# WesleyHsieh0806/TAO-Amodal

Hardware: AMD Instinct MI355X
Metric: box-pair IoU+match throughput (higher is better)
Workload: dtype f64

## Files before the change

### include/tao_amodal_hip.h

```cpp
#ifndef TAO_AMODAL_HIP_H
#define TAO_AMODAL_HIP_H

#include <stddef.h>
#include <stdint.h>

#ifdef __cplusplus
extern "C" {
#endif

#define TAOAMD_N_THR 10
#define TAOAMD_N_REC 101
#define TAOAMD_LVIS_RNG 6
#define TAOAMD_TAO_RNG 20

#define TAOAMD_GT_IGNORE 1
#define TAOAMD_GT_OOF 2
#define TAOAMD_GT_ID_HIDDEN 4
#define TAOAMD_DT_IGNORE_UNMATCHED 1
#define TAOAMD_DT_NO_CONSUME 2

#define TAOAMD_OK 0
#define TAOAMD_ERR_HIP 1
#define TAOAMD_ERR_ARG 2
#define TAOAMD_ERR_TOO_LARGE 3
// ... 59 lines not shown
                          const int32_t *gt_frame_pos, int64_t gt_frames,
                          int64_t gt_total, const int64_t *gt_off,
                          const uint32_t *gt_runs, const int32_t *gt_hw,
                          int32_t mode, double *iou,
                          int64_t *pair_frames, void *workspace,
                          size_t workspace_bytes, void *stream);

int taoamd_track_iou(int64_t n_cells, const int32_t *cell_dt_off,
                     const int32_t *cell_gt_off, const int64_t *cell_iou_off,
                     int64_t n_pairs, const int32_t *dt_frame_off,
                     const int32_t *dt_frame_pos, const double *dt_frame_box,
                     const int32_t *gt_frame_off, const int32_t *gt_frame_pos,
                     const double *gt_frame_box, int32_t mode, double *iou,
                     int64_t *pair_frames, void *stream);
int taoamd_track_iou_planned(int64_t n_tasks, const int32_t *tasks,
                             const int32_t *task_rows, const int32_t *task_pairs,
                             const int64_t *task_out, const double *frames,
                             const int32_t *task_base, const int32_t *trk_meta,
                             int32_t mode, double *iou, int64_t *pair_frames,
                             int64_t n_zero, const int64_t *zero_out,
                             void *stream);

int taoamd_track_iou_single(int64_t n_dt, const int32_t *dt_group,
                            const int64_t *cell_iou_off, const int32_t *dt_frame_pos,
                            const double *dt_frame_box, const int32_t *gt_frame_pos,
                            const double *gt_frame_box, int32_t mode, double *iou,
                            int64_t *pair_frames, void *stream);

int taoamd_track_pad(int64_t n_trk, int64_t n_frames, const int32_t *frame_off,
                     const int32_t *frame_pos, const double *frame_box,
                     const int32_t *meta, int64_t slot_first, int64_t n_slots,
                     double *padded, int32_t *inexact, void *stream);

int taoamd_track_stream(int64_t n_tasks, const int32_t *tasks,
                        const int32_t *task_rows, const int32_t *trk_meta,
                        const int32_t *task_base, const double *padded,
                        double *frames, void *stream);

int taoamd_track_iou_near(int64_t n_cells, const int32_t *cell_gt_off,
                          const int64_t *cell_iou_off, int64_t n_pairs,
                          const double *iou, int32_t max_ulp, int32_t capacity,
                          int32_t *count, int64_t *list, void *stream);

int64_t taoamd_track_iou_setorder_table(int64_t max_dt_frames, int64_t max_gt_frames);
int taoamd_track_iou_setorder(
    int64_t n_cells, const int32_t *cell_dt_off, const int32_t *cell_gt_off,
    const int64_t *cell_iou_off, const int32_t *cell_unit, const int64_t *tl_vid_start,
    const int64_t *tl_image_id, const int32_t *dt_frame_off, const int32_t *dt_frame_pos,
    const double *dt_frame_box, const int32_t *gt_frame_off, const int32_t *gt_frame_pos,
    const double *gt_frame_box, int32_t mode, const int32_t *count, int32_t capacity,
// ... 8 lines not shown
                                  const int64_t *b, int64_t *out, int64_t *n_out);

int taoamd_track_iou_plan_host(int64_t n_cells, const int32_t *cell_dt_off_host,
                               const int32_t *cell_gt_off_host,
                               const int64_t *cell_iou_off_host,
                               const int32_t *trk_meta_host, int64_t *sizes,
                               int32_t *tasks_host, int32_t *task_rows_host,
                               int32_t *task_pairs_host, int64_t *task_out_host);
int taoamd_track_iou_plan_spans_host(int64_t n_cells, const int32_t *cell_dt_off_host,
                                     const int32_t *cell_gt_off_host,
                                     const int64_t *cell_iou_off_host,
                                     const int32_t *trk_meta_host, int64_t *sizes,
                                     int32_t *tasks_host, int32_t *task_rows_host,
                                     int32_t *task_pairs_host, int64_t *task_out_host,
                                     int64_t *zero_out_host);

#define TAOAMD_MAX_GT_PER_CELL 3072
int taoamd_match(int64_t n_cells, const int32_t *cell_dt_off,
                 const int32_t *cell_gt_off, const int64_t *cell_iou_off,
                 int32_t max_gt_per_cell, const double *dt_box,
                 const double *gt_box, const double *iou, int32_t n_rng,
                 const uint32_t *gt_rng, const uint32_t *dt_rng,
                 const uint8_t *gt_flags, const uint8_t *dt_flags,
                 const int32_t *dst, int64_t out_stride, uint64_t *matched,
                 uint64_t *ignored, int32_t *match_gt, double *ious_out,
                 const int32_t *dt_group, const uint32_t *dt_meta,
                 const int32_t *groups, int32_t n_groups, const int32_t *singles,
                 int32_t n_singles, void *stream);

int taoamd_match_compact(int64_t n_cells, const int32_t *cell_dt_off,
// ... 422 lines not shown
```

### tao_amodal_amd/csrc/api.hip

```cpp
#include <stdio.h>
#include <string.h>

#include <map>
#include <mutex>
#include <string>
#include <vector>

#include "common.hpp"

namespace taoamd {

static thread_local char g_err[512] = "";

void set_error(hipError_t e, const char *what)
{
    snprintf(g_err, sizeof(g_err), "%s: %s", what, hipGetErrorString(e));
}

static void fill(double *out, double start, double stop, int num)
{
    const double step = (stop - start) / (double)(num - 1);
    for (int i = 0; i < num; i++) out[i] = (double)i * step + start;
    out[num - 1] = stop;
}
// ... 163 lines not shown

extern "C" const char *taoamd_strerror(int status)
{
    switch (status) {
    case TAOAMD_OK: return "ok";
    case TAOAMD_ERR_HIP: return "HIP runtime error (see taoamd_last_error)";
    case TAOAMD_ERR_ARG: return "bad argument";
    case TAOAMD_ERR_TOO_LARGE: return "a cell exceeds a kernel limit";
    case TAOAMD_ERR_WORKSPACE: return "workspace too small";
    }
    return "unknown status";
}

extern "C" const char *taoamd_last_error(void) { return taoamd::g_err; }

extern "C" int taoamd_version(void) { return 110; }

extern "C" int taoamd_thresholds_host(double *iou_thrs, double *rec_thrs)
{
    if (!iou_thrs || !rec_thrs) return TAOAMD_ERR_ARG;
    const IouThr i = taoamd::default_iou();
    const RecThr r = taoamd::default_rec();
    memcpy(iou_thrs, i.v, sizeof(double) * N_THR);
    memcpy(rec_thrs, r.v, sizeof(double) * N_REC);
    return TAOAMD_OK;
}

extern "C" int taoamd_set_thresholds(const double *iou_thrs, const double *rec_thrs)
{
    using namespace taoamd;
    IouThr i = default_iou();
// ... 40 lines not shown
```

### tao_amodal_amd/csrc/track_iou.hip

```cpp
#include <algorithm>
#include <vector>

#include "common.hpp"
#include "pyset.hpp"

using namespace taoamd;

__device__ __forceinline__ int64_t find_cell(const int64_t *__restrict__ off,
                                             int64_t n_cells, int64_t p)
{
    int64_t lo = 0, hi = n_cells;
    while (hi - lo > 1) {
        int64_t mid = (lo + hi) >> 1;
        if (off[mid] <= p) lo = mid; else hi = mid;
    }
    return lo;
}

struct FrameQueue {
    const int32_t *__restrict__ pos;
    const double4 *__restrict__ box;
    int32_t p, e;
    int32_t f0, f1, f2;
    double4 b0, b1, b2;
// ... 113 lines not shown
    }
    if (pair_frames != nullptr) {
        __shared__ unsigned long long s_common[4];
        for (int s = WAVE / 2; s > 0; s >>= 1)
            common += __shfl_down(common, s, WAVE);
        if (lane_id() == 0) s_common[threadIdx.x >> 6] = common;
        __syncthreads();
        if (threadIdx.x == 0) {
            const unsigned long long t = s_common[0] + s_common[1] + s_common[2] + s_common[3];
            if (t) atomicAdd(pair_frames, t);
        }
    }
}

#define TT_P 8
#define TT_ROWS 32
#define TT_RS (5 * TT_P + 2)
#define TT_GROUPS (64 / TT_P)
#define TT_ROUNDS ((TT_ROWS + TT_GROUPS - 1) / TT_GROUPS)
#define TT_SLOTS (TT_ROUNDS * TT_GROUPS)
#define TT_FAR 1e300
#define TT_SETS 2
#define TT_ZERO_PER 8

__device__ __forceinline__ double tt_max(double a, double b)
{
    double r;
    asm("v_max_f64 %0, %1, %2" : "=v"(r) : "v"(a), "v"(b));
    return r;
}
__device__ __forceinline__ double tt_min(double a, double b)
// ... 5 lines not shown
__device__ __forceinline__ double tt_pos(double a)
{
    double r;
    asm("v_max_f64 %0, %1, 0" : "=v"(r) : "v"(a));
    return r;
}

__device__ __forceinline__ void tt_barrier()
{
    asm volatile("s_waitcnt lgkmcnt(0)\n\ts_barrier" ::: "memory");
}

template <int S, bool MASKS>
__device__ __forceinline__ void tt_stager(
    const double4 *__restrict__ frames, int64_t sbase, double (*rows)[TT_ROWS * TT_RS],
    const int4 *meta, int32_t p_first, int n_chunks, int lane)
{
    constexpr int NR = (TT_ROUNDS - S + 1) / 2;
    const int grp = lane / TT_P, j = lane % TT_P;
    uint32_t bit[NR];
#pragma unroll
    for (int i = 0; i < NR; i++) bit[i] = 1u << (TT_GROUPS * (S + 2 * i) + grp);
    static_assert(TT_SLOTS <= 32, "one 32-bit mask of a task's rows");
    const int4 mrow = meta[lane & (TT_SLOTS - 1)];
    const uint32_t has_rows = (uint32_t)__builtin_amdgcn_ballot_w64(lane < TT_SLOTS && mrow.y >= mrow.x);
    double4 B[TT_SETS][NR];
    uint32_t pmv[TT_SETS];
    const char *const tbase = reinterpret_cast<const char *>(frames + sbase);
    uint32_t cur = 0;
    const uint32_t joff = (uint32_t)j * 32u;

    auto issue = [&](double4 *Bx, uint32_t &pm_set, int32_t pc) {
        const uint32_t pm = (uint32_t)(__builtin_amdgcn_ballot_w64(mrow.x < pc + TT_P) &
                                       __builtin_amdgcn_ballot_w64(mrow.y >= pc)) & has_rows;
        pm_set = pm;
#pragma unroll
        for (int i = 0; i < NR; i++) {
            const uint32_t off = cur + ((uint32_t)__popc(pm & (bit[i] - 1u)) << 8) + joff;
#ifdef TT_ABLATE_LOADS
            Bx[i] = *reinterpret_cast<const double4 *>(tbase + (off & 0u));
#elif defined(TT_ABLATE_CACHED)
            Bx[i] = *reinterpret_cast<const double4 *>(
                reinterpret_cast<const char *>(frames) + (((uint32_t)(sbase * 32) + off) & 0xfffe0u));
#else
            Bx[i] = *reinterpret_cast<const double4 *>(tbase + off);
#endif
        }
        cur += (uint32_t)__popc(pm) << 8;
    };
// ... 28 lines not shown
    for (int k = 0; k < n_chunks; k += TT_SETS) {
#pragma unroll
        for (int a = 1; a <= TT_SETS; a++) {
            const int c = k + a;
            if (c - 1 >= n_chunks) break;
            if (c < n_chunks) stage(B[a % TT_SETS], pmv[a % TT_SETS], a & 1);
            issue(B[a % TT_SETS], pmv[a % TT_SETS], p_first + (c + TT_SETS) * TT_P);
            tt_barrier();
        }
    }
}

template <int MODE, bool COUNT = true>
__global__ __launch_bounds__(192) __attribute__((amdgpu_waves_per_eu(MODE == 2 ? 4 : 6, MODE == 2 ? 4 : 6))) void track_iou_task_kernel(
    const int4 *__restrict__ tasks, const int32_t *__restrict__ task_rows,
    const int32_t *__restrict__ task_pairs, const int64_t *__restrict__ task_out,
    const double4 *__restrict__ frames, const int32_t *__restrict__ task_base,
    const int4 *__restrict__ trk_meta,
    double *__restrict__ iou, unsigned long long *__restrict__ pair_frames,
    int32_t n_tasks, int64_t n_zero, const int64_t *__restrict__ zero_out)
{
    __shared__ __align__(16) double rows[2][TT_ROWS * TT_RS];
    __shared__ int4 meta[TT_SLOTS];
    __shared__ int32_t span[2];

    if ((int32_t)blockIdx.x >= n_tasks) {
        const int64_t stride = (int64_t)(gridDim.x - n_tasks) * blockDim.x;
        for (int64_t k = (int64_t)(blockIdx.x - n_tasks) * blockDim.x + threadIdx.x;
             k < n_zero; k += stride)
            iou[zero_out[k]] = 0.0;
        return;
    }

    const int lane = threadIdx.x & 63;
    const int wave = threadIdx.x >> 6;
    const bool stager = wave < 2;
    const int4 tk = tasks[blockIdx.x];
    const int n_rows = tk.y, n_pairs = tk.w;

    if (wave == 0) {
        int32_t p_lo = INT32_MAX, p_hi = -1;
        if (lane < TT_SLOTS) {
            int4 m = make_int4(INT32_MAX, -1, 0, 0);
            if (lane < n_rows) m = trk_meta[task_rows[tk.x + lane]];
            if (m.y >= m.x) {
                p_lo = m.x;
                p_hi = m.y;
            } else {
                m.x = INT32_MAX;
                m.y = -1;
            }
            meta[lane] = m;
        }
#pragma unroll
        for (int s = 32; s > 0; s >>= 1) {
            p_lo = min(p_lo, __shfl_xor(p_lo, s));
            p_hi = max(p_hi, __shfl_xor(p_hi, s));
        }
        if (lane == 0) {
            span[0] = p_lo & ~(TT_P - 1);
            span[1] = p_hi;
        }
    }
    __syncthreads();
    const int32_t p_first = span[0], p_hi = span[1];
    const int n_chunks = p_hi < 0 ? 0 : (p_hi - p_first) / TT_P + 1;

    if (stager) {
        const int64_t sbase = (int64_t)task_base[blockIdx.x] * TT_P;
        constexpr bool MASKS = MODE != 0 || COUNT;
        if (wave == 0)
            tt_stager<0, MASKS>(frames, sbase, rows, meta, p_first, n_chunks, lane);
        else
            tt_stager<1, MASKS>(frames, sbase, rows, meta, p_first, n_chunks, lane);
        return;
    }

    int32_t pr = 0;
    if (lane < n_pairs) pr = task_pairs[tk.z + lane];
    const int rowd = pr & 0xFF, rowg = (pr >> 8) & 0xFF;
    int32_t Fd = INT32_MAX, Ld = -1, Fg = INT32_MAX, Lg = -1;
    if (lane < n_pairs) {
        const int4 md = meta[rowd], mg = meta[rowg];
        Fd = md.x;
        Ld = md.y;
        Fg = mg.x;
        Lg = mg.y;
    }
    const int offd = rowd * (TT_RS * 8), offg = rowg * (TT_RS * 8);
    double u = 0.0, i = 0.0;
    unsigned long long common = 0;
    auto add = [&](int b, int32_t pc) {
#ifdef TT_ABLATE_ADDER
        return;
#endif
        const bool dp = Fd < pc + TT_P && Ld >= pc;
        const bool gp = Fg < pc + TT_P && Lg >= pc;
        if (__ballot(dp || gp) == 0) return;
// ... 184 lines not shown
        const pyset::Frames D{dfpos + dfoff[td], dfbox + 4 * (int64_t)dfoff[td],
                              dfoff[td + 1] - dfoff[td]};
        const pyset::Frames Gf{gfpos + gfoff[tg], gfbox + 4 * (int64_t)gfoff[tg],
                               gfoff[tg + 1] - gfoff[tg]};
        if (pyset::table_size(4ull * ((uint64_t)D.n + Gf.n)) > table_cap) {
            atomicOr(status, 1);
            continue;
        }
        iou[p] = pyset::set_order_iou(tl_image_id + tl_vid_start[cell_unit[c]], D, Gf,
                                      mode, buf, table_cap);
    }
}

__global__ __launch_bounds__(TT_SLOTS * TT_P) void track_stream_kernel(
    const int4 *__restrict__ tasks, const int32_t *__restrict__ task_rows,
    const int4 *__restrict__ trk_meta, const int32_t *__restrict__ task_base,
    const double4 *__restrict__ padded, double4 *__restrict__ out)
{
    __shared__ int4 meta[TT_SLOTS];
    const int4 tk = tasks[blockIdx.x];
    const int tid = threadIdx.x;
    if (tid < TT_SLOTS)
        meta[tid] = tid < tk.y ? trk_meta[task_rows[tk.x + tid]] : make_int4(INT32_MAX, -1, 0, 0);
    if (blockIdx.x == 0 && tid < TT_P) out[tid] = make_double4(TT_FAR, TT_FAR, 0.0, 0.0);
    __syncthreads();
    int32_t p_lo = INT32_MAX, p_hi = -1;
    for (int r = 0; r < TT_SLOTS; r++) {
        const int4 m = meta[r];
        if (m.y >= m.x) {
            p_lo = min(p_lo, m.x);
            p_hi = max(p_hi, m.y);
        }
    }
    if (p_hi < 0) return;
    const int r = tid / TT_P, j = tid % TT_P;
    const int4 mine = meta[r];
    const bool has = mine.y >= mine.x;
    int64_t cursor = (int64_t)task_base[blockIdx.x] * TT_P;
    for (int32_t pc = p_lo & ~(TT_P - 1); pc <= p_hi; pc += TT_P) {
        uint32_t pm = 0;
        for (int q = 0; q < TT_SLOTS; q++) {
            const int4 m = meta[q];
            if (m.y >= m.x && m.x < pc + TT_P && m.y >= pc) pm |= 1u << q;
        }
        if (has && ((pm >> r) & 1u)) {
            const int32_t p = pc + j;
            const bool in = p >= mine.x && p <= mine.y;
            out[cursor + (__popc(pm & ((1u << r) - 1u)) * TT_P + j)] =
                in ? padded[(int64_t)mine.z + p] : make_double4(TT_FAR, TT_FAR, 0.0, 0.0);
        }
        cursor += __popc(pm) * TT_P;
    }
}

__global__ void track_pad_fill_kernel(int64_t n, double4 *__restrict__ padded)
{
    const int64_t k = blockIdx.x * (int64_t)blockDim.x + threadIdx.x;
    if (k < n) padded[k] = make_double4(TT_FAR, TT_FAR, 0.0, 0.0);
}

extern "C" int taoamd_track_iou(int64_t n_cells, const int32_t *cell_dt_off,
                                const int32_t *cell_gt_off,
                                const int64_t *cell_iou_off, int64_t n_pairs,
                                const int32_t *dt_frame_off,
                                const int32_t *dt_frame_pos,
                                const double *dt_frame_box,
// ... 28 lines not shown
    if (n_dt == 0) return TAOAMD_OK;
    if (!dt_group || !cell_iou_off || !dt_frame_pos || !dt_frame_box || !gt_frame_pos ||
        !gt_frame_box || !iou)
        return TAOAMD_ERR_ARG;
    TAO_TIMED("track_iou_single_kernel", s,
              track_iou_single_kernel<<<(unsigned)std::min<int64_t>((n_dt + 255) / 256, 2048), 256, 0, s>>>(
                  n_dt, (const int4 *)dt_group, cell_iou_off, dt_frame_pos,
                  (const double4 *)dt_frame_box, gt_frame_pos, (const double4 *)gt_frame_box,
                  iou, (unsigned long long *)pair_frames, mode));
    TAO_LAUNCH_CHECK();
    return TAOAMD_OK;
}

extern "C" int taoamd_track_iou_planned(int64_t n_tasks, const int32_t *tasks,
                                        const int32_t *task_rows,
                                        const int32_t *task_pairs,
                                        const int64_t *task_out,
                                        const double *frames,
                                        const int32_t *task_base,
                                        const int32_t *trk_meta, int32_t mode,
                                        double *iou, int64_t *pair_frames,
                                        int64_t n_zero, const int64_t *zero_out,
                                        void *stream)
{
    hipStream_t s = (hipStream_t)stream;
    if (mode < 0 || mode > 2 || n_tasks < 0 || n_tasks > INT32_MAX - 4096 || n_zero < 0 ||
        (n_zero > 0 && !zero_out))
        return TAOAMD_ERR_ARG;
    if (pair_frames) TAO_HIP(hipMemsetAsync(pair_frames, 0, 8, s));
    if (n_tasks == 0 && n_zero == 0) return TAOAMD_OK;
    if (!iou || (n_tasks > 0 && (!tasks || !task_rows || !task_pairs || !task_out || !frames ||
                                 !task_base || !trk_meta)))
        return TAOAMD_ERR_ARG;
    unsigned long long *pf = (unsigned long long *)pair_frames;
    const unsigned zero_wgs = (unsigned)std::min<int64_t>(
        (n_zero + 192 * TT_ZERO_PER - 1) / (192 * TT_ZERO_PER), 4096);
    const unsigned grid = (unsigned)n_tasks + zero_wgs;
    static const unsigned lds_pad = getenv("TAOAMD_TT_LDS_PAD") ? (unsigned)atoi(getenv("TAOAMD_TT_LDS_PAD")) : 0u;
#define TT_LAUNCH(M)                                                           \
    TAO_TIMED("track_iou_task_kernel", s,                                      \
              track_iou_task_kernel<M><<<grid, 192, lds_pad, s>>>(             \
                  (const int4 *)tasks, task_rows, task_pairs, task_out,        \
                  (const double4 *)frames, task_base, (const int4 *)trk_meta, iou, pf, \
                  (int32_t)n_tasks, n_zero, zero_out))
    if (mode == 0 && pf == nullptr)
        TAO_TIMED("track_iou_task_kernel", s,
                  (track_iou_task_kernel<0, false><<<grid, 192, lds_pad, s>>>(
                      (const int4 *)tasks, task_rows, task_pairs, task_out,
                      (const double4 *)frames, task_base, (const int4 *)trk_meta, iou, pf,
                      (int32_t)n_tasks, n_zero, zero_out)));
    else if (mode == 0) TT_LAUNCH(0);
    else if (mode == 1) TT_LAUNCH(1);
    else TT_LAUNCH(2);
#undef TT_LAUNCH
    TAO_LAUNCH_CHECK();
    return TAOAMD_OK;
}

extern "C" int taoamd_track_pad(int64_t n_trk, int64_t n_frames,
                                const int32_t *frame_off,
                                const int32_t *frame_pos,
                                const double *frame_box, const int32_t *meta,
                                int64_t slot_first, int64_t n_slots,
// ... 7 lines not shown
        TAO_TIMED("track_pad_fill_kernel", s, track_pad_fill_kernel<<<(unsigned)((n_slots + 255) / 256), 256, 0, s>>>(
            n_slots, (double4 *)padded + slot_first));
    }
    if (n_frames > 0) {
        if (!frame_off || !frame_pos || !frame_box || !meta || !padded)
            return TAOAMD_ERR_ARG;
        TAO_TIMED("track_pad_kernel", s, track_pad_kernel<<<(unsigned)((n_frames + 255) / 256), 256, 0, s>>>(
            n_frames, n_trk, frame_off, frame_pos, (const double4 *)frame_box,
            (const int4 *)meta, (double4 *)padded, inexact));
    }
    TAO_LAUNCH_CHECK();
    return TAOAMD_OK;
}

extern "C" int taoamd_track_stream(int64_t n_tasks, const int32_t *tasks,
                                   const int32_t *task_rows, const int32_t *trk_meta,
                                   const int32_t *task_base, const double *padded,
                                   double *frames, void *stream)
{
    hipStream_t s = (hipStream_t)stream;
    if (n_tasks < 0) return TAOAMD_ERR_ARG;
    if (n_tasks == 0) return TAOAMD_OK;
    if (!tasks || !task_rows || !trk_meta || !task_base || !padded || !frames)
        return TAOAMD_ERR_ARG;
    TAO_TIMED("track_stream_kernel", s,
              track_stream_kernel<<<(unsigned)n_tasks, TT_SLOTS * TT_P, 0, s>>>(
                  (const int4 *)tasks, task_rows, (const int4 *)trk_meta, task_base,
                  (const double4 *)padded, (double4 *)frames));
    TAO_LAUNCH_CHECK();
    return TAOAMD_OK;
}

extern "C" int taoamd_track_iou_near(int64_t n_cells, const int32_t *cell_gt_off,
                                     const int64_t *cell_iou_off, int64_t n_pairs,
                                     const double *iou, int32_t max_ulp,
                                     int32_t capacity, int32_t *count,
                                     int64_t *list, void *stream)
{
    hipStream_t s = (hipStream_t)stream;
    if (n_cells < 0 || n_pairs < 0 || max_ulp < 0 || capacity < 0 || !count)
        return TAOAMD_ERR_ARG;
    TAO_HIP(hipMemsetAsync(count, 0, sizeof(int32_t), s));
// ... 85 lines not shown
    }
    const uint32_t cap = pyset::table_size(4ull * (uint64_t)(n_a + n_b));
    std::vector<int32_t> buf(3 * (size_t)cap);
    auto hash = [&](int32_t c) { return (uint64_t)keys[c - 1]; };
    auto ca = [&](uint32_t k) { return code[k]; };
    auto cb = [&](uint32_t k) { return code[n_a + k]; };
    const pyset::Set R = pyset::set_union((uint32_t)n_a, ca, (uint32_t)n_b, cb, hash,
                                          buf.data(), cap);
    int64_t n = 0;
    for (uint32_t i = 0; i <= R.mask; i++)
        if (R.t[i]) out[n++] = keys[R.t[i] - 1];
    *n_out = n;
    return TAOAMD_OK;
}

static int tt_plan(bool spans, int64_t n_cells, const int32_t *cell_dt_off,
                   const int32_t *cell_gt_off, const int64_t *cell_iou_off,
                   const int32_t *trk_meta, int64_t *sizes, int32_t *tasks,
                   int32_t *task_rows, int32_t *task_pairs, int64_t *task_out,
                   int64_t *zero_out)
{
    if (n_cells < 0 || !cell_dt_off || !cell_gt_off || !cell_iou_off ||
        !trk_meta || !sizes)
        return TAOAMD_ERR_ARG;
    const bool fill = tasks != nullptr;
    if (fill && (!task_rows || !task_pairs || !task_out)) return TAOAMD_ERR_ARG;
    const int64_t n_dt = cell_dt_off[n_cells];
    auto first_of = [&](int64_t t) { return trk_meta[4 * t]; };
    auto last_of = [&](int64_t t) { return trk_meta[4 * t + 1]; };
    auto zero_pair = [&](int64_t d, int64_t g) {
// ... 19 lines not shown
        for (int64_t c = 0; c < n_cells; c++) {
            if (cell_hi[c] < 0) continue;
            const int32_t d0 = cell_dt_off[c], D = cell_dt_off[c + 1] - d0;
            const int32_t g0 = cell_gt_off[c], G = cell_gt_off[c + 1] - g0;
            for (int32_t d = 0; d < D; d++)
                for (int32_t g = 0; g < G; g++)
                    if (zero_pair(d0 + d, n_dt + g0 + g)) {
                        if (zero_out) zero_out[nz] = cell_iou_off[c] + (int64_t)d * G + g;
                        nz++;
                    }
        }
    std::stable_sort(order.begin(), order.end(), [&](int64_t a, int64_t b) {
        return cell_hi[a] > cell_hi[b];
    });
    int64_t nt = 0, nr = 0, np = 0;
    int32_t rows[TT_ROWS], n_rows = 0, n_pairs = 0;
    int32_t pair_d[64], pair_g[64];
    int64_t pair_out[64];
    auto close = [&]() {
        if (n_pairs == 0) { n_rows = 0; return; }
        if (fill) {
            int32_t perm[TT_ROWS], inv[TT_ROWS];
            for (int r = 0; r < n_rows; r++) perm[r] = r;
            std::stable_sort(perm, perm + n_rows, [&](int32_t a, int32_t b) {
                return first_of(rows[a]) < first_of(rows[b]);
            });
            for (int r = 0; r < n_rows; r++) inv[perm[r]] = r;
            tasks[4 * nt] = (int32_t)nr;
            tasks[4 * nt + 1] = n_rows;
            tasks[4 * nt + 2] = (int32_t)np;
            tasks[4 * nt + 3] = n_pairs;
            for (int r = 0; r < n_rows; r++) task_rows[nr + r] = rows[perm[r]];
            for (int k = 0; k < n_pairs; k++) {
                task_pairs[np + k] = inv[pair_d[k]] | (inv[pair_g[k]] << 8);
                task_out[np + k] = pair_out[k];
            }
        }
        nt++;
        nr += n_rows;
        np += n_pairs;
        n_rows = n_pairs = 0;
    };
    std::vector<int32_t> dts;
    for (int64_t c : order) {
        const int32_t d0 = cell_dt_off[c], D = cell_dt_off[c + 1] - d0;
        const int32_t g0 = cell_gt_off[c], G = cell_gt_off[c + 1] - g0;
        dts.resize(D);
        for (int32_t d = 0; d < D; d++) dts[d] = d;
        std::stable_sort(dts.begin(), dts.end(), [&](int32_t a, int32_t b) {
            return first_of(d0 + a) < first_of(d0 + b);
        });
        const int32_t gblocks = (G + TT_ROWS - 2) / (TT_ROWS - 1);
        for (int32_t gb = 0; gb < gblocks; gb++) {
            const int32_t ga = (int32_t)((int64_t)gb * G / gblocks);
            const int32_t ng = (int32_t)((int64_t)(gb + 1) * G / gblocks) - ga;
            int32_t grow[TT_ROWS];
            std::fill(grow, grow + ng, -1);
            for (int32_t k = 0; k < D; k++) {
                const int32_t d = dts[k];
                int32_t keep[TT_ROWS], nk = 0, fresh = 0;
                for (int32_t g = 0; g < ng; g++)
                    if (!zero_pair(d0 + d, n_dt + g0 + ga + g)) {
                        keep[nk++] = g;
                        fresh += grow[g] < 0;
                    }
                if (nk == 0) continue;
                int32_t drow = -1;
                for (int32_t r = 0; gb > 0 && r < n_rows; r++)
                    if (rows[r] == d0 + d) drow = r;
                if (n_pairs + nk > 64 || n_rows + fresh + (drow < 0) > TT_ROWS) {
                    close();
                    std::fill(grow, grow + ng, -1);
                    fresh = nk;
                    drow = -1;
                }
                for (int32_t j = 0; j < nk; j++)
                    if (grow[keep[j]] < 0) {
                        grow[keep[j]] = n_rows;
                        rows[n_rows++] = (int32_t)(n_dt + g0 + ga + keep[j]);
                    }
                if (drow < 0) {
                    drow = n_rows;
                    rows[n_rows++] = d0 + d;
                }
                for (int32_t j = 0; j < nk; j++) {
// ... 20 lines not shown
    int32_t *tasks, int32_t *task_rows, int32_t *task_pairs, int64_t *task_out)
{
    return tt_plan(false, n_cells, cell_dt_off, cell_gt_off, cell_iou_off, trk_meta, sizes,
                   tasks, task_rows, task_pairs, task_out, nullptr);
}

extern "C" int taoamd_track_iou_plan_spans_host(
    int64_t n_cells, const int32_t *cell_dt_off, const int32_t *cell_gt_off,
    const int64_t *cell_iou_off, const int32_t *trk_meta, int64_t *sizes,
    int32_t *tasks, int32_t *task_rows, int32_t *task_pairs, int64_t *task_out,
    int64_t *zero_out)
{
    return tt_plan(true, n_cells, cell_dt_off, cell_gt_off, cell_iou_off, trk_meta, sizes,
                   tasks, task_rows, task_pairs, task_out, zero_out);
}
```

### tao_amodal_amd/engine.py

```python
import os

import numpy as np
import torch

from . import _lib

N_THR, N_REC = _lib.N_THR, _lib.N_REC


def _ptr(t):
    return None if t is None else t.data_ptr()


def _stream():
    return torch.cuda.current_stream().cuda_stream


def _to_device(v, device):
    from .flatten import LazyRows
    if not isinstance(v, LazyRows):
        return torch.from_numpy(np.ascontiguousarray(v)).to(device)
    from .flatten_dev import device_copy
    src = device_copy(v.source, device)
    if len(v.index) == 0:
# ... 93 lines not shown
            np.zeros(int(sizes[2]), dtype=np.int32),
            np.zeros(int(sizes[2]), dtype=np.int64)]
    if spans:
        tabs.append(np.zeros(int(sizes[3]), dtype=np.int64))
    if sizes[0] or (spans and sizes[3]):
        _lib.check(getattr(lib, name)(*args, *(t.ctypes.data for t in tabs)), name)
    return tuple(tabs)


def track_iou_plan(flat, meta):
    return _track_iou_plan(flat, meta, False)


def track_iou_plan_spans(flat, meta):
    return _track_iou_plan(flat, meta, True)


class DeviceProblem:

    IOU_MODES = {"3d_iou": 0, "avg_iou": 1, "imagenetvid": 2}

    def __init__(self, flat, device="cuda", iou_3d_type="3d_iou", guard="device"):
        self.kind = flat.kind
        self.iou_mode = self.IOU_MODES[iou_3d_type]
        self.device = torch.device(device)
        self.n_rng = _lib.LVIS_RNG if self.kind == "lvis" else _lib.TAO_RNG
        self.n_words = (self.n_rng * N_THR + 63) // 64
        self.n_cells = int(flat.n_cells)
        self.n_cat = len(flat.cat_ids)
        self.n_dt = int(flat.cell_dt_off[-1])
# ... 130 lines not shown
        if self.mask_iou:
            return
        meta, sides, n_slots = track_meta(flat)
        n_frames = sum(int(getattr(flat, "dev", {})[k].numel())
                       if k in getattr(flat, "dev", {}) and not dict.__contains__(flat, k)
                       else len(flat[k]) for k in ("dt_frame_pos", "gt_frame_pos"))
        self.n_slots = n_slots
        if n_slots > 4 * n_frames + (1 << 20) or n_slots >= 2 ** 31 - 1:
            return
        self.single_frame = (len(meta) > 0 and n_frames == len(meta)
                             and bool((meta[:, 0] == meta[:, 1]).all())
                             and os.environ.get("TAOAMD_SINGLE_FRAME", "1") != "0")
        if self.single_frame:
            self.exact_terms = True
            return
        tasks, rows, pairs, out, zero = track_iou_plan_spans(flat, meta)
        self.n_tasks = len(tasks)
        if self.n_tasks == 0:
            return
        dev = self.device
        self.t["tasks"] = torch.from_numpy(tasks).to(dev)
        self.t["task_rows"] = torch.from_numpy(rows).to(dev)
        self.t["task_pairs"] = torch.from_numpy(pairs).to(dev)
        self.t["task_out"] = torch.from_numpy(out).to(dev)
        self.t["zero_out"] = torch.from_numpy(zero).to(dev)
        self.t["trk_meta"] = torch.from_numpy(
            np.ascontiguousarray(meta, dtype=np.int32)).to(dev)
        padded = torch.empty((n_slots, 4), dtype=torch.float64, device=dev)
        n_dt = int(self.t["dt_frame_off"].numel()) - 1
        inexact = torch.zeros(1, dtype=torch.int32, device=dev)
        with torch.cuda.device(dev):
            for side, row0 in (("dt", 0), ("gt", n_dt)):
                slot0, slots = sides[side]
                n_trk = int(self.t[side + "_frame_off"].numel()) - 1
                _lib.check(lib.taoamd_track_pad(
                    n_trk, int(self.t[side + "_frame_pos"].numel()),
                    _ptr(self.t[side + "_frame_off"]),
# ... 4 lines not shown
                    "taoamd_track_pad")
            has = meta[:, 1] >= meta[:, 0]
            trk_pieces = np.where(has, (meta[:, 1] >> 3) - (meta[:, 0] >> 3) + 1, 0)
            task_pieces = np.add.reduceat(trk_pieces[rows].astype(np.int64),
                                          tasks[:, 0].astype(np.int64))
            base = 1 + np.cumsum(task_pieces) - task_pieces
            n_pieces = 1 + int(task_pieces.sum())
            if n_pieces >= 2 ** 31 - 1 or int(task_pieces.max()) * 256 >= 2 ** 32:
                self._drop_plan()
                return
            self.t["task_base"] = torch.from_numpy(base.astype(np.int32)).to(dev)
            self.t["frames"] = torch.empty(((n_pieces + 64) * 8, 4), dtype=torch.float64,
                                           device=dev)
            _lib.check(lib.taoamd_track_stream(
                self.n_tasks, _ptr(self.t["tasks"]), _ptr(self.t["task_rows"]),
                _ptr(self.t["trk_meta"]), _ptr(self.t["task_base"]), _ptr(padded),
                _ptr(self.t["frames"]), _stream()), "taoamd_track_stream")
            del padded
        longest = int((meta[:, 1] - meta[:, 0]).max()) + 1 if len(meta) else 0
        flags = int(inexact.item())
        self.exact_terms = not (flags & 1) and longest <= 4096
        if flags & 2:
            self._drop_plan()

    PLAN_TABLES = ("tasks", "task_rows", "task_pairs", "task_out", "frames",
                   "task_base", "trk_meta", "zero_out")

    def _drop_plan(self):
        for k in self.PLAN_TABLES:
            self.t[k] = None

    def guard_active(self):
        return (self.kind == "tao" and self.n_iou > 0 and self.iou_mode != 2
                and not self.mask_iou
                and not (self.exact_terms and self.iou_mode == 0)
                and not self.single_frame and self.device.type == "cuda")

    def _plan_guard(self, flat, guard):
        if not self.guard_active():
            return
# ... 247 lines not shown
    if dp.kind != "tao" or dp.n_iou == 0:
        return
    if dp.mask_iou:
        return stage_track_mask_iou(dp, ws)
    lib, t, s = _lib.load(), dp.t, _stream()
    if dp.single_frame:
        _lib.check(lib.taoamd_track_iou_single(
            dp.n_dt, _ptr(t["dt_group"]), _ptr(t["cell_iou_off"]),
            _ptr(t["dt_frame_pos"]), _ptr(t["dt_frame_box"]), _ptr(t["gt_frame_pos"]),
            _ptr(t["gt_frame_box"]), dp.iou_mode, _ptr(ws.iou), _ptr(ws.pair_frames), s),
            "taoamd_track_iou_single")
        return
    if t["tasks"] is not None:
        counted = ws.pairs_counted and dp.iou_mode == 0
        _lib.check(lib.taoamd_track_iou_planned(
            dp.n_tasks, _ptr(t["tasks"]), _ptr(t["task_rows"]),
            _ptr(t["task_pairs"]), _ptr(t["task_out"]), _ptr(t["frames"]),
            _ptr(t["task_base"]), _ptr(t["trk_meta"]), dp.iou_mode, _ptr(ws.iou),
            None if counted else _ptr(ws.pair_frames), int(t["zero_out"].numel()),
            _ptr(t["zero_out"]), s), "taoamd_track_iou_planned")
        ws.pairs_counted = True
        return
    _lib.check(lib.taoamd_track_iou(
        dp.n_cells, _ptr(t["cell_dt_off"]), _ptr(t["cell_gt_off"]),
        _ptr(t["cell_iou_off"]), dp.n_iou, _ptr(t["dt_frame_off"]),
        _ptr(t["dt_frame_pos"]), _ptr(t["dt_frame_box"]),
        _ptr(t["gt_frame_off"]), _ptr(t["gt_frame_pos"]),
        _ptr(t["gt_frame_box"]), dp.iou_mode, _ptr(ws.iou),
        _ptr(ws.pair_frames), s), "taoamd_track_iou")


# ... 772 lines not shown
```

Baseline: 47080.

## Pack up to 64 tracks per task by chaining temporally disjoint tracks into shared row slots

Adds a host-side packer that regroups planned tasks so each task holds up to 64 tracks while only 32 staging rows are live at once. Tracks whose frame spans do not overlap share a row slot through a per-slot linked list (head and next indices in task_slots), and the stager and stream kernels advance along that list as the frame cursor moves. The aim is more pairs per task and fewer tasks and frame chunks for the same shared-memory footprint. In exchange the stream kernel gains extra syncthreads per chunk, the stager does more shared-memory meta lookups, and host planning gets more complex.

```diff
diff --git a/include/tao_amodal_hip.h b/include/tao_amodal_hip.h
--- a/include/tao_amodal_hip.h
+++ b/include/tao_amodal_hip.h
@@ -97,7 +97,8 @@
                      const double *gt_frame_box, int32_t mode, double *iou,
                      int64_t *pair_frames, void *stream);
 int taoamd_track_iou_planned(int64_t n_tasks, const int32_t *tasks,
-                             const int32_t *task_rows, const int32_t *task_pairs,
+                             const int32_t *task_rows, const int32_t *task_slots,
+                             const int32_t *task_pairs,
                              const int64_t *task_out, const double *frames,
                              const int32_t *task_base, const int32_t *trk_meta,
                              int32_t mode, double *iou, int64_t *pair_frames,
@@ -116,7 +117,8 @@
                      double *padded, int32_t *inexact, void *stream);
 
 int taoamd_track_stream(int64_t n_tasks, const int32_t *tasks,
-                        const int32_t *task_rows, const int32_t *trk_meta,
+                        const int32_t *task_rows, const int32_t *task_slots,
+                        const int32_t *trk_meta,
                         const int32_t *task_base, const double *padded,
                         double *frames, void *stream);
 
@@ -155,6 +157,16 @@
                                      int32_t *tasks_host, int32_t *task_rows_host,
                                      int32_t *task_pairs_host, int64_t *task_out_host,
                                      int64_t *zero_out_host);
+
+int taoamd_track_iou_limits(int32_t *limits);
+int taoamd_track_iou_pack_host(int64_t n_tasks, const int32_t *tasks_host,
+                               const int32_t *task_rows_host,
+                               const int32_t *task_pairs_host,
+                               const int64_t *task_out_host,
+                               const int32_t *trk_meta_host, int32_t max_tracks,
+                               int32_t max_live, int64_t *sizes, int32_t *tasks_out,
+                               int32_t *task_rows_out, int32_t *task_slots_out,
+                               int32_t *task_pairs_out, int64_t *task_out_out);
 
 #define TAOAMD_MAX_GT_PER_CELL 3072
 int taoamd_match(int64_t n_cells, const int32_t *cell_dt_off,
diff --git a/tao_amodal_amd/csrc/api.hip b/tao_amodal_amd/csrc/api.hip
--- a/tao_amodal_amd/csrc/api.hip
+++ b/tao_amodal_amd/csrc/api.hip
@@ -201,7 +201,7 @@
 
 extern "C" const char *taoamd_last_error(void) { return taoamd::g_err; }
 
-extern "C" int taoamd_version(void) { return 110; }
+extern "C" int taoamd_version(void) { return 111; }
 
 extern "C" int taoamd_thresholds_host(double *iou_thrs, double *rec_thrs)
 {
diff --git a/tao_amodal_amd/csrc/track_iou.hip b/tao_amodal_amd/csrc/track_iou.hip
--- a/tao_amodal_amd/csrc/track_iou.hip
+++ b/tao_amodal_amd/csrc/track_iou.hip
@@ -151,7 +151,10 @@
 }
 
 #define TT_P 8
+#ifndef TT_ROWS
 #define TT_ROWS 32
+#endif
+#define TT_TRACKS 64
 #define TT_RS (5 * TT_P + 2)
 #define TT_GROUPS (64 / TT_P)
 #define TT_ROUNDS ((TT_ROWS + TT_GROUPS - 1) / TT_GROUPS)
@@ -187,7 +190,7 @@
 template <int S, bool MASKS>
 __device__ __forceinline__ void tt_stager(
     const double4 *__restrict__ frames, int64_t sbase, double (*rows)[TT_ROWS * TT_RS],
-    const int4 *meta, int32_t p_first, int n_chunks, int lane)
+    const int4 *meta, const int32_t *head, int32_t p_first, int n_chunks, int lane)
 {
     constexpr int NR = (TT_ROUNDS - S + 1) / 2;
     const int grp = lane / TT_P, j = lane % TT_P;
@@ -195,8 +198,8 @@
 #pragma unroll
     for (int i = 0; i < NR; i++) bit[i] = 1u << (TT_GROUPS * (S + 2 * i) + grp);
     static_assert(TT_SLOTS <= 32, "one 32-bit mask of a task's rows");
-    const int4 mrow = meta[lane & (TT_SLOTS - 1)];
-    const uint32_t has_rows = (uint32_t)__builtin_amdgcn_ballot_w64(lane < TT_SLOTS && mrow.y >= mrow.x);
+    int4 mrow = meta[lane < TT_SLOTS ? head[lane] : TT_TRACKS];
+    int4 mnext = meta[mrow.z];
     double4 B[TT_SETS][NR];
     uint32_t pmv[TT_SETS];
     const char *const tbase = reinterpret_cast<const char *>(frames + sbase);
@@ -204,8 +207,13 @@
     const uint32_t joff = (uint32_t)j * 32u;
 
     auto issue = [&](double4 *Bx, uint32_t &pm_set, int32_t pc) {
+        if (mrow.y < pc && mnext.y >= 0) {
+            mrow.x = mnext.x;
+            mrow.y = mnext.y;
+            mnext = meta[mnext.z];
+        }
         const uint32_t pm = (uint32_t)(__builtin_amdgcn_ballot_w64(mrow.x < pc + TT_P) &
-                                       __builtin_amdgcn_ballot_w64(mrow.y >= pc)) & has_rows;
+                                       __builtin_amdgcn_ballot_w64(mrow.y >= pc));
         pm_set = pm;
 #pragma unroll
         for (int i = 0; i < NR; i++) {
@@ -264,6 +272,7 @@
 template <int MODE, bool COUNT = true>
 __global__ __launch_bounds__(192) __attribute__((amdgpu_waves_per_eu(MODE == 2 ? 4 : 6, MODE == 2 ? 4 : 6))) void track_iou_task_kernel(
     const int4 *__restrict__ tasks, const int32_t *__restrict__ task_rows,
+    const int32_t *__restrict__ task_slots,
     const int32_t *__restrict__ task_pairs, const int64_t *__restrict__ task_out,
     const double4 *__restrict__ frames, const int32_t *__restrict__ task_base,
     const int4 *__restrict__ trk_meta,
@@ -271,7 +280,8 @@
     int32_t n_tasks, int64_t n_zero, const int64_t *__restrict__ zero_out)
 {
     __shared__ __align__(16) double rows[2][TT_ROWS * TT_RS];
-    __shared__ int4 meta[TT_SLOTS];
+    __shared__ int4 meta[TT_TRACKS + 1];
+    __shared__ int32_t head[TT_SLOTS];
     __shared__ int32_t span[2];
 
     if ((int32_t)blockIdx.x >= n_tasks) {
@@ -290,18 +300,21 @@
 
     if (wave == 0) {
         int32_t p_lo = INT32_MAX, p_hi = -1;
-        if (lane < TT_SLOTS) {
-            int4 m = make_int4(INT32_MAX, -1, 0, 0);
-            if (lane < n_rows) m = trk_meta[task_rows[tk.x + lane]];
-            if (m.y >= m.x) {
-                p_lo = m.x;
-                p_hi = m.y;
-            } else {
-                m.x = INT32_MAX;
-                m.y = -1;
-            }
-            meta[lane] = m;
-        }
+        static_assert(TT_TRACKS == 64, "a lane per track");
+        int4 m = make_int4(INT32_MAX, -1, TT_TRACKS, 0);
+        if (lane < TT_SLOTS) head[lane] = TT_TRACKS;
+        if (lane < n_rows) {
+            const int4 t = trk_meta[task_rows[tk.x + lane]];
+            const int32_t w = task_slots[tk.x + lane];
+            if (t.y >= t.x) {
+                p_lo = m.x = t.x;
+                p_hi = m.y = t.y;
+                m.z = min((w >> 8) & 0xFF, TT_TRACKS);
+                if (w & 0x10000) head[min(w & 0xFF, TT_SLOTS - 1)] = lane;
+            }
+        }
+        meta[lane] = m;
+        if (lane == 0) meta[TT_TRACKS] = make_int4(INT32_MAX, -1, TT_TRACKS, 0);
 #pragma unroll
         for (int s = 32; s > 0; s >>= 1) {
             p_lo = min(p_lo, __shfl_xor(p_lo, s));
@@ -320,18 +333,19 @@
         const int64_t sbase = (int64_t)task_base[blockIdx.x] * TT_P;
         constexpr bool MASKS = MODE != 0 || COUNT;
         if (wave == 0)
-            tt_stager<0, MASKS>(frames, sbase, rows, meta, p_first, n_chunks, lane);
+            tt_stager<0, MASKS>(frames, sbase, rows, meta, head, p_first, n_chunks, lane);
         else
-            tt_stager<1, MASKS>(frames, sbase, rows, meta, p_first, n_chunks, lane);
+            tt_stager<1, MASKS>(frames, sbase, rows, meta, head, p_first, n_chunks, lane);
         return;
     }
 
     int32_t pr = 0;
     if (lane < n_pairs) pr = task_pairs[tk.z + lane];
-    const int rowd = pr & 0xFF, rowg = (pr >> 8) & 0xFF;
+    const int trkd = pr & (TT_TRACKS - 1), trkg = (pr >> 8) & (TT_TRACKS - 1);
+    const int rowd = min((pr >> 16) & 0xFF, TT_ROWS - 1), rowg = min((pr >> 24) & 0xFF, TT_ROWS - 1);
     int32_t Fd = INT32_MAX, Ld = -1, Fg = INT32_MAX, Lg = -1;
     if (lane < n_pairs) {
-        const int4 md = meta[rowd], mg = meta[rowg];
+        const int4 md = meta[trkd], mg = meta[trkg];
         Fd = md.x;
         Ld = md.y;
         Fg = mg.x;
@@ -546,19 +560,34 @@
 
 __global__ __launch_bounds__(TT_SLOTS * TT_P) void track_stream_kernel(
     const int4 *__restrict__ tasks, const int32_t *__restrict__ task_rows,
+    const int32_t *__restrict__ task_slots,
     const int4 *__restrict__ trk_meta, const int32_t *__restrict__ task_base,
     const double4 *__restrict__ padded, double4 *__restrict__ out)
 {
-    __shared__ int4 meta[TT_SLOTS];
+    static_assert(TT_SLOTS * TT_P > TT_TRACKS, "a thread per track and one more");
+    __shared__ int4 meta[TT_TRACKS + 1];
+    __shared__ int32_t occ[TT_SLOTS];
     const int4 tk = tasks[blockIdx.x];
     const int tid = threadIdx.x;
-    if (tid < TT_SLOTS)
-        meta[tid] = tid < tk.y ? trk_meta[task_rows[tk.x + tid]] : make_int4(INT32_MAX, -1, 0, 0);
+    if (tid < TT_SLOTS) occ[tid] = TT_TRACKS;
     if (blockIdx.x == 0 && tid < TT_P) out[tid] = make_double4(TT_FAR, TT_FAR, 0.0, 0.0);
     __syncthreads();
+    if (tid <= TT_TRACKS) {
+        int4 m = make_int4(INT32_MAX, -1, 0, TT_TRACKS);
+        if (tid < tk.y && tid < TT_TRACKS) {
+            const int4 t = trk_meta[task_rows[tk.x + tid]];
+            const int32_t w = task_slots[tk.x + tid];
+            if (t.y >= t.x) {
+                m = make_int4(t.x, t.y, t.z, min((w >> 8) & 0xFF, TT_TRACKS));
+                if (w & 0x10000) occ[min(w & 0xFF, TT_SLOTS - 1)] = tid;
+            }
+        }
+        meta[tid] = m;
+    }
+    __syncthreads();
     int32_t p_lo = INT32_MAX, p_hi = -1;
-    for (int r = 0; r < TT_SLOTS; r++) {
-        const int4 m = meta[r];
+    for (int t = 0; t < TT_TRACKS; t++) {
+        const int4 m = meta[t];
         if (m.y >= m.x) {
             p_lo = min(p_lo, m.x);
             p_hi = max(p_hi, m.y);
@@ -566,22 +595,27 @@
     }
     if (p_hi < 0) return;
     const int r = tid / TT_P, j = tid % TT_P;
-    const int4 mine = meta[r];
-    const bool has = mine.y >= mine.x;
     int64_t cursor = (int64_t)task_base[blockIdx.x] * TT_P;
     for (int32_t pc = p_lo & ~(TT_P - 1); pc <= p_hi; pc += TT_P) {
+        if (tid < TT_SLOTS) {
+            const int4 m = meta[occ[tid]];
+            if (m.y < pc && meta[m.w].y >= 0) occ[tid] = m.w;
+        }
+        __syncthreads();
         uint32_t pm = 0;
         for (int q = 0; q < TT_SLOTS; q++) {
-            const int4 m = meta[q];
-            if (m.y >= m.x && m.x < pc + TT_P && m.y >= pc) pm |= 1u << q;
-        }
-        if (has && ((pm >> r) & 1u)) {
+            const int4 m = meta[occ[q]];
+            if (m.x < pc + TT_P && m.y >= pc) pm |= 1u << q;
+        }
+        if ((pm >> r) & 1u) {
+            const int4 mine = meta[occ[r]];
             const int32_t p = pc + j;
             const bool in = p >= mine.x && p <= mine.y;
             out[cursor + (__popc(pm & ((1u << r) - 1u)) * TT_P + j)] =
                 in ? padded[(int64_t)mine.z + p] : make_double4(TT_FAR, TT_FAR, 0.0, 0.0);
         }
         cursor += __popc(pm) * TT_P;
+        __syncthreads();
     }
 }
 
@@ -640,6 +674,7 @@
 
 extern "C" int taoamd_track_iou_planned(int64_t n_tasks, const int32_t *tasks,
                                         const int32_t *task_rows,
+                                        const int32_t *task_slots,
                                         const int32_t *task_pairs,
                                         const int64_t *task_out,
                                         const double *frames,
@@ -655,7 +690,7 @@
         return TAOAMD_ERR_ARG;
     if (pair_frames) TAO_HIP(hipMemsetAsync(pair_frames, 0, 8, s));
     if (n_tasks == 0 && n_zero == 0) return TAOAMD_OK;
-    if (!iou || (n_tasks > 0 && (!tasks || !task_rows || !task_pairs || !task_out || !frames ||
+    if (!iou || (n_tasks > 0 && (!tasks || !task_rows || !task_slots || !task_pairs || !task_out || !frames ||
                                  !task_base || !trk_meta)))
         return TAOAMD_ERR_ARG;
     unsigned long long *pf = (unsigned long long *)pair_frames;
@@ -666,13 +701,13 @@
 #define TT_LAUNCH(M)                                                           \
     TAO_TIMED("track_iou_task_kernel", s,                                      \
               track_iou_task_kernel<M><<<grid, 192, lds_pad, s>>>(             \
-                  (const int4 *)tasks, task_rows, task_pairs, task_out,        \
+                  (const int4 *)tasks, task_rows, task_slots, task_pairs, task_out,        \
                   (const double4 *)frames, task_base, (const int4 *)trk_meta, iou, pf, \
                   (int32_t)n_tasks, n_zero, zero_out))
     if (mode == 0 && pf == nullptr)
         TAO_TIMED("track_iou_task_kernel", s,
                   (track_iou_task_kernel<0, false><<<grid, 192, lds_pad, s>>>(
-                      (const int4 *)tasks, task_rows, task_pairs, task_out,
+                      (const int4 *)tasks, task_rows, task_slots, task_pairs, task_out,
                       (const double4 *)frames, task_base, (const int4 *)trk_meta, iou, pf,
                       (int32_t)n_tasks, n_zero, zero_out)));
     else if (mode == 0) TT_LAUNCH(0);
@@ -710,18 +745,19 @@
 }
 
 extern "C" int taoamd_track_stream(int64_t n_tasks, const int32_t *tasks,
-                                   const int32_t *task_rows, const int32_t *trk_meta,
+                                   const int32_t *task_rows, const int32_t *task_slots,
+                                   const int32_t *trk_meta,
                                    const int32_t *task_base, const double *padded,
                                    double *frames, void *stream)
 {
     hipStream_t s = (hipStream_t)stream;
     if (n_tasks < 0) return TAOAMD_ERR_ARG;
     if (n_tasks == 0) return TAOAMD_OK;
-    if (!tasks || !task_rows || !trk_meta || !task_base || !padded || !frames)
+    if (!tasks || !task_rows || !task_slots || !trk_meta || !task_base || !padded || !frames)
         return TAOAMD_ERR_ARG;
     TAO_TIMED("track_stream_kernel", s,
               track_stream_kernel<<<(unsigned)n_tasks, TT_SLOTS * TT_P, 0, s>>>(
-                  (const int4 *)tasks, task_rows, (const int4 *)trk_meta, task_base,
+                  (const int4 *)tasks, task_rows, task_slots, (const int4 *)trk_meta, task_base,
                   (const double4 *)padded, (double4 *)frames));
     TAO_LAUNCH_CHECK();
     return TAOAMD_OK;
@@ -837,6 +873,8 @@
     return TAOAMD_OK;
 }
 
+#define TT_PLAN_ROWS 32
+static_assert(TT_PLAN_ROWS <= TT_TRACKS, "a task of the plan is a task of the packer");
 static int tt_plan(bool spans, int64_t n_cells, const int32_t *cell_dt_off,
                    const int32_t *cell_gt_off, const int64_t *cell_iou_off,
                    const int32_t *trk_meta, int64_t *sizes, int32_t *tasks,
@@ -886,13 +924,13 @@
         return cell_hi[a] > cell_hi[b];
     });
     int64_t nt = 0, nr = 0, np = 0;
-    int32_t rows[TT_ROWS], n_rows = 0, n_pairs = 0;
+    int32_t rows[TT_PLAN_ROWS], n_rows = 0, n_pairs = 0;
     int32_t pair_d[64], pair_g[64];
     int64_t pair_out[64];
     auto close = [&]() {
         if (n_pairs == 0) { n_rows = 0; return; }
         if (fill) {
-            int32_t perm[TT_ROWS], inv[TT_ROWS];
+            int32_t perm[TT_PLAN_ROWS], inv[TT_PLAN_ROWS];
             for (int r = 0; r < n_rows; r++) perm[r] = r;
             std::stable_sort(perm, perm + n_rows, [&](int32_t a, int32_t b) {
                 return first_of(rows[a]) < first_of(rows[b]);
@@ -922,15 +960,15 @@
         std::stable_sort(dts.begin(), dts.end(), [&](int32_t a, int32_t b) {
             return first_of(d0 + a) < first_of(d0 + b);
         });
-        const int32_t gblocks = (G + TT_ROWS - 2) / (TT_ROWS - 1);
+        const int32_t gblocks = (G + TT_PLAN_ROWS - 2) / (TT_PLAN_ROWS - 1);
         for (int32_t gb = 0; gb < gblocks; gb++) {
             const int32_t ga = (int32_t)((int64_t)gb * G / gblocks);
             const int32_t ng = (int32_t)((int64_t)(gb + 1) * G / gblocks) - ga;
-            int32_t grow[TT_ROWS];
+            int32_t grow[TT_PLAN_ROWS];
             std::fill(grow, grow + ng, -1);
             for (int32_t k = 0; k < D; k++) {
                 const int32_t d = dts[k];
-                int32_t keep[TT_ROWS], nk = 0, fresh = 0;
+                int32_t keep[TT_PLAN_ROWS], nk = 0, fresh = 0;
                 for (int32_t g = 0; g < ng; g++)
                     if (!zero_pair(d0 + d, n_dt + g0 + ga + g)) {
                         keep[nk++] = g;
@@ -940,7 +978,7 @@
                 int32_t drow = -1;
                 for (int32_t r = 0; gb > 0 && r < n_rows; r++)
                     if (rows[r] == d0 + d) drow = r;
-                if (n_pairs + nk > 64 || n_rows + fresh + (drow < 0) > TT_ROWS) {
+                if (n_pairs + nk > 64 || n_rows + fresh + (drow < 0) > TT_PLAN_ROWS) {
                     close();
                     std::fill(grow, grow + ng, -1);
                     fresh = nk;
@@ -991,3 +1029,162 @@
     return tt_plan(true, n_cells, cell_dt_off, cell_gt_off, cell_iou_off, trk_meta, sizes,
                    tasks, task_rows, task_pairs, task_out, zero_out);
 }
+
+extern "C" int taoamd_track_iou_limits(int32_t *limits)
+{
+    if (!limits) return TAOAMD_ERR_ARG;
+    limits[0] = TT_ROWS;
+    limits[1] = TT_TRACKS;
+    limits[2] = 64;
+    limits[3] = TT_P;
+    return TAOAMD_OK;
+}
+
+extern "C" int taoamd_track_iou_pack_host(
+    int64_t n_tasks, const int32_t *tasks, const int32_t *task_rows,
+    const int32_t *task_pairs, const int64_t *task_out, const int32_t *trk_meta,
+    int32_t max_tracks, int32_t max_live, int64_t *sizes, int32_t *tasks_out,
+    int32_t *rows_out, int32_t *slots_out, int32_t *pairs_out, int64_t *out_out)
+{
+    if (n_tasks < 0 || !sizes || max_live < 1 || max_live > TT_ROWS || max_tracks < max_live ||
+        max_tracks > TT_TRACKS)
+        return TAOAMD_ERR_ARG;
+    if (n_tasks > 0 && (!tasks || !task_rows || !task_pairs || !task_out || !trk_meta))
+        return TAOAMD_ERR_ARG;
+    const bool fill = tasks_out != nullptr;
+    if (fill && (!rows_out || !slots_out || !pairs_out || !out_out)) return TAOAMD_ERR_ARG;
+    auto first_of = [&](int64_t t) { return trk_meta[4 * t]; };
+    auto last_of = [&](int64_t t) { return trk_meta[4 * t + 1]; };
+    auto has_frames = [&](int64_t t) { return first_of(t) <= last_of(t); };
+    int32_t n_chunks = 0;
+    for (int64_t k = 0; k < n_tasks; k++) {
+        const int32_t r0 = tasks[4 * k], nr_ = tasks[4 * k + 1], np_ = tasks[4 * k + 3];
+        if (r0 < 0 || nr_ < 0 || nr_ > TT_TRACKS || tasks[4 * k + 2] < 0 || np_ < 0 || np_ > 64)
+            return TAOAMD_ERR_ARG;
+        for (int32_t r = 0; r < nr_; r++) {
+            const int64_t t = task_rows[r0 + r];
+            if (t < 0 || (has_frames(t) && first_of(t) < 0)) return TAOAMD_ERR_ARG;
+            if (has_frames(t)) n_chunks = std::max(n_chunks, (last_of(t) >> 3) + 1);
+        }
+    }
+    std::vector<int32_t> live(n_chunks, 0);
+    int64_t nt = 0, nr = 0, np = 0;
+    int32_t trk[TT_TRACKS], n_trk = 0, n_pairs = 0;
+    int64_t seen[TT_TRACKS];
+    int32_t pair_d[64], pair_g[64];
+    int64_t pair_out[64];
+    auto close = [&]() -> int {
+        if (n_pairs == 0) return TAOAMD_OK;
+        if (fill) {
+            int32_t perm[TT_TRACKS], inv[TT_TRACKS];
+            for (int r = 0; r < n_trk; r++) perm[r] = r;
+            std::sort(perm, perm + n_trk, [&](int32_t a, int32_t b) {
+                const int32_t fa = first_of(trk[a]), fb = first_of(trk[b]);
+                return fa != fb ? fa < fb : seen[a] < seen[b];
+            });
+            for (int r = 0; r < n_trk; r++) inv[perm[r]] = r;
+            int32_t row_end[TT_ROWS], row_last[TT_ROWS], row_of[TT_TRACKS];
+            std::fill(row_end, row_end + TT_ROWS, -1);
+            std::fill(row_last, row_last + TT_ROWS, -1);
+            for (int r = 0; r < n_trk; r++) {
+                const int32_t t = trk[perm[r]];
+                rows_out[nr + r] = t;
+                row_of[r] = 0;
+                if (!has_frames(t)) {
+                    slots_out[nr + r] = 0xFF | (TT_TRACKS << 8);
+                    continue;
+                }
+                int32_t s = 0;
+                while (s < max_live && row_end[s] >= (first_of(t) >> 3)) s++;
+                if (s == max_live) return TAOAMD_ERR_ARG;
+                const bool head = row_last[s] < 0;
+                if (!head)
+                    slots_out[nr + row_last[s]] =
+                        (slots_out[nr + row_last[s]] & ~0xFF00) | (r << 8);
+                slots_out[nr + r] = s | (TT_TRACKS << 8) | (head ? 0x10000 : 0);
+                row_end[s] = last_of(t) >> 3;
+                row_last[s] = r;
+                row_of[r] = s;
+            }
+            tasks_out[4 * nt] = (int32_t)nr;
+            tasks_out[4 * nt + 1] = n_trk;
+            tasks_out[4 * nt + 2] = (int32_t)np;
+            tasks_out[4 * nt + 3] = n_pairs;
+            for (int k = 0; k < n_pairs; k++) {
+                const int32_t d = inv[pair_d[k]], g = inv[pair_g[k]];
+                pairs_out[np + k] = d | (g << 8) | (row_of[d] << 16) | (row_of[g] << 24);
+                out_out[np + k] = pair_out[k];
+            }
+        }
+        for (int r = 0; r < n_trk; r++)
+            if (has_frames(trk[r]))
+                for (int32_t c = first_of(trk[r]) >> 3; c <= (last_of(trk[r]) >> 3); c++) live[c]--;
+        nt++;
+        nr += n_trk;
+        np += n_pairs;
+        n_trk = n_pairs = 0;
+        return TAOAMD_OK;
+    };
+    auto find = [&](int32_t t) {
+        for (int r = 0; r < n_trk; r++)
+            if (trk[r] == t) return r;
+        return -1;
+    };
+    auto join = [&](int32_t t, int64_t at) {
+        if (n_trk == max_tracks) return false;
+        if (has_frames(t)) {
+            const int32_t c0 = first_of(t) >> 3, c1 = last_of(t) >> 3;
+            for (int32_t c = c0; c <= c1; c++)
+                if (live[c] >= max_live) return false;
+            for (int32_t c = c0; c <= c1; c++) live[c]++;
+        }
+        trk[n_trk] = t;
+        seen[n_trk++] = at;
+        return true;
+    };
+    auto leave = [&]() {
+        const int32_t t = trk[--n_trk];
+        if (has_frames(t))
+            for (int32_t c = first_of(t) >> 3; c <= (last_of(t) >> 3); c++) live[c]--;
+    };
+    for (int64_t k = 0; k < n_tasks; k++) {
+        const int32_t r0 = tasks[4 * k], p0 = tasks[4 * k + 2], np_ = tasks[4 * k + 3];
+        const int32_t nr_ = tasks[4 * k + 1];
+        for (int32_t a = 0; a < np_;) {
+            const int32_t od = task_pairs[p0 + a] & 0xFF;
+            int32_t b = a + 1;
+            while (b < np_ && (task_pairs[p0 + b] & 0xFF) == od) b++;
+            if (od >= nr_) return TAOAMD_ERR_ARG;
+            for (int attempt = 0;; attempt++) {
+                const int32_t before = n_trk;
+                bool fits = n_pairs + (b - a) <= 64;
+                for (int32_t q = a; q <= b && fits; q++) {
+                    const int32_t orow = q < b ? (task_pairs[p0 + q] >> 8) & 0xFF : od;
+                    if (orow >= nr_) return TAOAMD_ERR_ARG;
+                    const int32_t t = task_rows[r0 + orow];
+                    if (find(t) < 0) fits = join(t, k * 256 + orow);
+                }
+                if (fits) break;
+                while (n_trk > before) leave();
+                if (attempt == 1) return TAOAMD_ERR_ARG;
+                const int st = close();
+                if (st != TAOAMD_OK) return st;
+            }
+            const int32_t d = find(task_rows[r0 + od]);
+            for (int32_t q = a; q < b; q++) {
+                pair_d[n_pairs] = d;
+                pair_g[n_pairs] = find(task_rows[r0 + ((task_pairs[p0 + q] >> 8) & 0xFF)]);
+                pair_out[n_pairs] = task_out[p0 + q];
+                n_pairs++;
+            }
+            a = b;
+        }
+    }
+    const int st = close();
+    if (st != TAOAMD_OK) return st;
+    if (nr >= INT32_MAX || np >= INT32_MAX) return TAOAMD_ERR_ARG;
+    sizes[0] = nt;
+    sizes[1] = nr;
+    sizes[2] = np;
+    return TAOAMD_OK;
+}
diff --git a/tao_amodal_amd/engine.py b/tao_amodal_amd/engine.py
--- a/tao_amodal_amd/engine.py
+++ b/tao_amodal_amd/engine.py
@@ -131,6 +131,38 @@
 
 def track_iou_plan_spans(flat, meta):
     return _track_iou_plan(flat, meta, True)
+
+
+def track_iou_limits():
+    lim = np.zeros(4, dtype=np.int32)
+    _lib.check(_lib.load().taoamd_track_iou_limits(lim.ctypes.data), "taoamd_track_iou_limits")
+    return tuple(int(v) for v in lim)
+
+
+def track_iou_pack(plan, meta, max_tracks=None, max_live=None):
+    lib = _lib.load()
+    rows_cap, tracks_cap = track_iou_limits()[:2]
+    max_tracks = tracks_cap if max_tracks is None else int(max_tracks)
+    max_live = rows_cap if max_live is None else int(max_live)
+    tasks, rows, pairs, out = (np.ascontiguousarray(a, dtype=t) for a, t in zip(
+        plan[:4], (np.int32, np.int32, np.int32, np.int64)))
+    meta = np.ascontiguousarray(meta, dtype=np.int32)
+    sizes = np.zeros(3, dtype=np.int64)
+    args = (len(tasks), tasks.ctypes.data, rows.ctypes.data, pairs.ctypes.data,
+            out.ctypes.data, meta.ctypes.data, max_tracks, max_live, sizes.ctypes.data)
+    name = "taoamd_track_iou_pack_host"
+    _lib.check(getattr(lib, name)(*args, *([None] * 5)), name)
+    tabs = [np.zeros((int(sizes[0]), 4), dtype=np.int32),
+            np.zeros(int(sizes[1]), dtype=np.int32),
+            np.zeros(int(sizes[1]), dtype=np.int32),
+            np.zeros(int(sizes[2]), dtype=np.int32),
+            np.zeros(int(sizes[2]), dtype=np.int64)]
+    if sizes[0]:
+        _lib.check(getattr(lib, name)(*args, *(t.ctypes.data for t in tabs)), name)
+    return tuple(tabs)
+
+
+TRACK_PACK_LIMITS = (None, None)
 
 
 class DeviceProblem:
@@ -291,13 +323,16 @@
         if self.single_frame:
             self.exact_terms = True
             return
-        tasks, rows, pairs, out, zero = track_iou_plan_spans(flat, meta)
+        plan = track_iou_plan_spans(flat, meta)
+        zero = plan[4]
+        tasks, rows, slots, pairs, out = track_iou_pack(plan, meta, *TRACK_PACK_LIMITS)
         self.n_tasks = len(tasks)
         if self.n_tasks == 0:
             return
         dev = self.device
         self.t["tasks"] = torch.from_numpy(tasks).to(dev)
         self.t["task_rows"] = torch.from_numpy(rows).to(dev)
+        self.t["task_slots"] = torch.from_numpy(slots).to(dev)
         self.t["task_pairs"] = torch.from_numpy(pairs).to(dev)
         self.t["task_out"] = torch.from_numpy(out).to(dev)
         self.t["zero_out"] = torch.from_numpy(zero).to(dev)
@@ -332,6 +367,7 @@
                                            device=dev)
             _lib.check(lib.taoamd_track_stream(
                 self.n_tasks, _ptr(self.t["tasks"]), _ptr(self.t["task_rows"]),
+                _ptr(self.t["task_slots"]),
                 _ptr(self.t["trk_meta"]), _ptr(self.t["task_base"]), _ptr(padded),
                 _ptr(self.t["frames"]), _stream()), "taoamd_track_stream")
             del padded
@@ -341,7 +377,7 @@
         if flags & 2:
             self._drop_plan()
 
-    PLAN_TABLES = ("tasks", "task_rows", "task_pairs", "task_out", "frames",
+    PLAN_TABLES = ("tasks", "task_rows", "task_slots", "task_pairs", "task_out", "frames",
                    "task_base", "trk_meta", "zero_out")
 
     def _drop_plan(self):
@@ -619,7 +655,7 @@
     if t["tasks"] is not None:
         counted = ws.pairs_counted and dp.iou_mode == 0
         _lib.check(lib.taoamd_track_iou_planned(
-            dp.n_tasks, _ptr(t["tasks"]), _ptr(t["task_rows"]),
+            dp.n_tasks, _ptr(t["tasks"]), _ptr(t["task_rows"]), _ptr(t["task_slots"]),
             _ptr(t["task_pairs"]), _ptr(t["task_out"]), _ptr(t["frames"]),
             _ptr(t["task_base"]), _ptr(t["trk_meta"]), dp.iou_mode, _ptr(ws.iou),
             None if counted else _ptr(ws.pair_frames), int(t["zero_out"].numel()),
```

Measured after the change: 47540, median of 6. No clear change (+1.0%).
